# imironhead/ml_super_resolution

Hardware: AMD Instinct MI355X
Metric: VDSR-20 training patches/sec (41x41, batch 256 per GPU); fwd HR megapixels/sec alongside (higher is better)
Workload: dtype f32; 1 GPU; BASELINE configs[2]: VDSR 20-layer 3x3x64 residual, RGB, batch 256x41x41 per GPU, fwd+bwd+TF-Adam, random-init weights; global_batch=256, patch=41, parallelism=dp1

## Files before the change

### include/srx.h

```cpp
#ifndef SRX_H_
#define SRX_H_

#include <stddef.h>
#include <stdint.h>

#ifdef __cplusplus
extern "C" {
#endif

typedef void* srx_stream_t;

typedef enum {
    SRX_OK = 0,
    SRX_ERR_BAD_ARG = -1,
    SRX_ERR_UNSUPPORTED = -2,
    SRX_ERR_WORKSPACE = -3,
    SRX_ERR_LAUNCH = -4,
    SRX_ERR_ALIGN = -5
} srx_status;

typedef enum { SRX_PAD_SAME = 0, SRX_PAD_VALID = 1 } srx_pad_mode;

typedef enum {
    SRX_ACT_NONE = 0,
// ... 17 lines not shown
    int32_t subpixel_r;
} srx_conv_desc;

const char* srx_version(void);
const char* srx_last_error(void);

int srx_set_conv_path(int pipelined);

int srx_set_wgrad_path(int path);

int srx_conv_chain(const srx_conv_desc* d, int op, int in_act, int layers, const float* const* x, const float* const* w,
                   const float* const* bias, const float* const* aux, float* const* y, srx_stream_t stream);

int srx_conv_chain_supported(const srx_conv_desc* d, int op, int in_act);

int srx_set_chain(int on);

int srx_conv2d_precision_supported(const srx_conv_desc* d, int op);

size_t srx_conv2d_workspace_bytes(const srx_conv_desc* d, int op);

int srx_conv2d_fwd(const srx_conv_desc* d, const float* x, const float* w, const float* bias,
                   const float* skip, float* y, void* ws, size_t ws_bytes, srx_stream_t stream);

int srx_conv2d_bwd_data(const srx_conv_desc* d, const float* dpre, const float* w,
                        const float* x_in, int in_act, float* dx_out, void* ws, size_t ws_bytes,
                        srx_stream_t stream);

int srx_conv2d_bwd_data_acc(const srx_conv_desc* d, const float* dpre, const float* w, const float* dx_acc,
                            float* dx_out, void* ws, size_t ws_bytes, srx_stream_t stream);

// ... 163 lines not shown
```

### ml_super_resolution_amd/_lib.py

```python
import ctypes
import os

_HERE = os.path.dirname(os.path.abspath(__file__))
LIB_PATH = os.path.join(_HERE, 'libsrx.so')

SRX_OK = 0
PAD_SAME, PAD_VALID = 0, 1
ACT_NONE, ACT_RELU, ACT_TANH, ACT_LRELU, ACT_SIGMOID = 0, 1, 2, 3, 4
OP_FWD, OP_BWD_DATA, OP_BWD_FILTER = 0, 1, 2
PRECISION_FP32, PRECISION_BF16X3 = 0, 1
PRECISION_BY_NAME = {'highest': PRECISION_FP32, 'high': PRECISION_BF16X3}

ACT_BY_NAME = {None: ACT_NONE, 'none': ACT_NONE, 'relu': ACT_RELU, 'tanh': ACT_TANH,
               'lrelu': ACT_LRELU, 'leaky_relu': ACT_LRELU, 'sigmoid': ACT_SIGMOID}
PAD_BY_NAME = {'same': PAD_SAME, 'valid': PAD_VALID}

EXPORTS = [
    'srx_version', 'srx_last_error', 'srx_set_conv_path', 'srx_set_wgrad_path', 'srx_set_chain', 'srx_conv_chain', 'srx_conv_chain_supported', 'srx_conv2d_precision_supported', 'srx_conv2d_workspace_bytes', 'srx_conv2d_fwd',
    'srx_conv2d_bwd_data', 'srx_conv2d_bwd_filter', 'srx_conv2d_bwd_filter_partials', 'srx_conv2d_bwd_filter_reduce', 'srx_act_bwd', 'srx_depth_to_space',
    'srx_space_to_depth', 'srx_stream_copy', 'srx_mse_fwd_bwd', 'srx_l2_loss', 'srx_reduce_scratch_bytes',
    'srx_adam_tf_step', 'srx_adam_tf_step_dev', 'srx_momentum_clip_step', 'srx_rownorm_loss_fwd_bwd', 'srx_psnr', 'srx_ssim', 'srx_ssim_scratch_bytes', 'srx_saturate_u8', 'srx_affine', 'srx_u8_to_unit_float', 'srx_gaussian_blur', 'srx_resize_bilinear',
    'srx_upsample_nearest', 'srx_upsample_nearest_bwd', 'srx_add_relu_grad',
    'srx_conv2d_bwd_data_acc', 'srx_conv3x3_blocked', 'srx_conv3x3_blocked_bwd_filter_workspace_bytes', 'srx_conv3x3_blocked_bwd_filter',
    'srx_conv3x3_blocked_ex', 'srx_conv3x3_blocked_bwd_filter_ex_workspace_bytes', 'srx_conv3x3_blocked_bwd_filter_ex',
    'srx_espcn_forward', 'srx_espcn_forward_keep', 'srx_debug_poison_lds', 'srx_srcnn_forward', 'srx_maxpool2x2', 'srx_maxpool2x2_bwd', 'srx_maxpool2x2_bwd_masked', 'srx_subsample2', 'srx_subsample2_bwd',
    'srx_channel_blocks_to_nhwc', 'srx_nhwc_to_channel_blocks', 'srx_channel_normalize', 'srx_channel_normalize_bwd',
    'srx_extract_patches16', 'srx_texture_gram', 'srx_texture_gram_bwd', 'srx_pil_resample_ksize', 'srx_pil_resample_coeffs', 'srx_resample_u8', 'srx_u8_to_pm1', 'srx_log_loss', 'srx_vgg_preprocess', 'srx_add_scaled', 'srx_resize_bicubic_tf', 'srx_column_sums', 'srx_gemm_workspace_bytes', 'srx_gemm',
]


class SrxError(RuntimeError):
    pass

# ... 22 lines not shown
    if not os.path.exists(LIB_PATH):
        raise SrxError('libsrx.so not found at %s -- build it with `make -C %s` (or '
                       '__graft_entry__.build()); there is no CPU fallback' %
                       (LIB_PATH, os.path.join(_HERE, 'csrc')))
    import torch
    L = ctypes.CDLL(LIB_PATH)
    vp, sz, i, f = ctypes.c_void_p, ctypes.c_size_t, ctypes.c_int, ctypes.c_float
    dp = ctypes.POINTER(ConvDesc)
    L.srx_version.restype = ctypes.c_char_p
    L.srx_last_error.restype = ctypes.c_char_p
    L.srx_set_conv_path.argtypes = [i]
    L.srx_set_wgrad_path.argtypes = [i]
    L.srx_set_chain.argtypes = [i]
    L.srx_conv_chain_supported.argtypes = [dp, i, i]
    L.srx_conv_chain.argtypes = [dp, i, i, i, vp, vp, vp, vp, vp, vp]
    L.srx_conv2d_precision_supported.argtypes = [dp, i]
    L.srx_conv2d_workspace_bytes.argtypes = [dp, i]
    L.srx_conv2d_workspace_bytes.restype = sz
    L.srx_reduce_scratch_bytes.restype = sz
    L.srx_conv2d_fwd.argtypes = [dp, vp, vp, vp, vp, vp, vp, sz, vp]
    L.srx_conv2d_bwd_data.argtypes = [dp, vp, vp, vp, i, vp, vp, sz, vp]
    L.srx_conv2d_bwd_filter.argtypes = [dp, vp, vp, vp, vp, vp, f, vp, sz, vp]
    L.srx_conv2d_bwd_filter_partials.argtypes = [dp, vp, vp, vp, sz, ctypes.POINTER(ctypes.c_int), vp]
    L.srx_conv2d_bwd_filter_reduce.argtypes = [dp, vp, i, vp, vp, vp, f, vp]
    L.srx_act_bwd.argtypes = [vp, vp, vp, sz, i, vp]
    L.srx_depth_to_space.argtypes = [vp, vp, i, i, i, i, i, vp]
    L.srx_space_to_depth.argtypes = [vp, vp, i, i, i, i, i, vp]
    L.srx_stream_copy.argtypes = [vp, vp, sz, vp]
    L.srx_mse_fwd_bwd.argtypes = [vp, vp, sz, f, vp, i, vp, vp, vp]
    L.srx_l2_loss.argtypes = [vp, vp, sz, f, vp, i, vp, vp]
# ... 63 lines not shown
```

### ml_super_resolution_amd/csrc/conv_chain.hip

```cpp
#include "launchers.h"
namespace srx {

template <bool WT, int AUX>
__global__ __launch_bounds__(256, 1) void conv_chain_kernel(const ConvArgs a, const ChainPtrs c) {
    for (int l = 0; l < c.L; ++l) {
        ConvArgs al = a;
        al.x = c.x[l]; al.w = c.w[l]; al.bias = c.bias[l]; al.y = c.y[l];
        if (WT) al.mask = c.aux[l];
        else al.skip = c.aux[l];
        asm volatile("" : "+s"(al.N), "+s"(al.H), "+s"(al.W), "+s"(al.OH), "+s"(al.OW), "+s"(al.Cin), "+s"(al.Cout));
        asm volatile("" : "+s"(al.pad_t), "+s"(al.pad_l), "+s"(al.TH), "+s"(al.TW), "+s"(al.NTX), "+s"(al.RS));
        asm volatile("" : "+s"(al.units_total), "+s"(al.act), "+s"(al.post_relu), "+s"(al.mask_act), "+s"(al.buf_floats));
        conv_pipe_body<3, 3, 64, 4, WT, AUX, false>(al, l == 0);
        asm volatile("s_waitcnt vmcnt(0)" ::: "memory");
        __builtin_amdgcn_fence(__ATOMIC_RELEASE, "workgroup");
        __builtin_amdgcn_s_barrier();
        __builtin_amdgcn_fence(__ATOMIC_ACQUIRE, "workgroup");
    }
}

hipError_t launch_conv_chain(bool wt, bool aux, const ConvArgs& a, const ChainPtrs& c, int grid, size_t lds, hipStream_t s) {
    if (!wt) return aux ? hipErrorInvalidValue : launch_chain_with_lds(conv_chain_kernel<false, 0>, a, c, grid, lds, s);
    return aux ? launch_chain_with_lds(conv_chain_kernel<true, 1>, a, c, grid, lds, s)
               : launch_chain_with_lds(conv_chain_kernel<true, 0>, a, c, grid, lds, s);
}
}
```

### ml_super_resolution_amd/csrc/conv_kernels.hip.h

```cpp
#pragma once
#include <hip/hip_runtime.h>
#include <stdint.h>
#include <type_traits>

namespace srx {

typedef float f32x4 __attribute__((ext_vector_type(4)));

enum { ACT_NONE = 0, ACT_RELU = 1, ACT_TANH = 2, ACT_LRELU = 3, ACT_SIGMOID = 4 };

struct ConvArgs {
    const float* x;
    const float* w;
    const float* bias;
    const float* skip;
    const float* mask;
    float* y;
    int N, H, W, OH, OW, Cin, Cout;
    int pad_t, pad_l;
    int TH, TW, NTX, RS;
    int units_total;
    int act, post_relu, mask_act;
    float inv_rs;
    int stagger;
// ... 19 lines not shown
    float inv_rs;
    int stagger;
    int zero_slot;
    int stride;
    unsigned long long* trace;
};

constexpr int kChainMax = 32;
struct ChainPtrs {
    const float* x[kChainMax];
    const float* w[kChainMax];
    const float* bias[kChainMax];
    const float* aux[kChainMax];
    float* y[kChainMax];
    int L;
};

template <int CINP>
struct Lds {
    static constexpr int PS = (CINP == 4) ? 4 : CINP + 4;
};

__device__ __forceinline__ float srx_tanhf(float x) {
    const float ax = fabsf(x);
    const float x2 = ax * ax;
    float p = fmaf(x2, -0.006274174898862839f, 0.021071631461381912f);
    p = fmaf(x2, p, -0.053852297365665436f);
    p = fmaf(x2, p, 0.13332585990428925f);
    p = fmaf(x2, p, -0.33333316445350647f);
    const float small = fmaf(x2 * ax, p, ax);
// ... 2415 lines not shown
        }
    }
    bsum += __shfl_xor(bsum, 16);
    bsum += __shfl_xor(bsum, 32);
    if (qpart == 0 && kq == 0 && co_ok) pw[(size_t)TAPS * a.Cin * a.Cout + co] = bsum;
}

template <int IMM>
__device__ __forceinline__ float dpre_fire_imm(__amdgpu_buffer_rsrc_t rsrc, int voff, int soff) {
    float b;
    asm volatile("buffer_load_dword %0, %1, %2, %3 offen offset:%4" : "=&a"(b) : "v"(voff), "s"(rsrc), "s"(soff), "n"(IMM) : "memory");
    return b;
}

template <int KH, int KW, int CINP, int NCH, int OWC>
__global__ __launch_bounds__(256, 1) void wgrad_rows_full_kernel(const WgradArgs a) {
    extern __shared__ __attribute__((aligned(16))) float lds[];
    constexpr int PS = Lds<CINP>::PS;
    constexpr int TAPS = KH * KW;
    constexpr int ROWS = TAPS * CINP;
    constexpr int Q = (ROWS + 63) / 64;
    constexpr int NQP = 4 / NCH;
    constexpr int QW = (Q + NQP - 1) / NQP;
    constexpr int TPP = CINP / 4, PPP = 256 / TPP;
    constexpr int SPR = OWC / 4;
    constexpr int THC = 3;
    constexpr int RSZ = OWC + 1;
    constexpr int COUTC = 64;
    constexpr int U = THC * SPR + 1;
    constexpr int JP = (RSZ + PPP - 1) / PPP;
    constexpr int NPASSES = (THC + KH - 1) * JP;
// ... 229 lines not shown
#pragma unroll
        for (int g = 0; g < 4; ++g) {
#pragma unroll
            for (int r = 0; r < 4; ++r) {
                const int R = 64 * q + 4 * (4 * kq + r) + g;
                const int tap = R / CINP, ci = R % CINP;
                if (R < ROWS && ci < a.Cin && co_ok) pw[((size_t)tap * a.Cin + ci) * a.Cout + co] = acc[k][g][r];
            }
        }
    }
    bsum += __shfl_xor(bsum, 16);
    bsum += __shfl_xor(bsum, 32);
    if (qpart == 0 && kq == 0 && co_ok) pw[(size_t)TAPS * a.Cin * a.Cout + co] = bsum;
}

}
```

### ml_super_resolution_amd/csrc/launchers.h

```cpp
#pragma once
#include "conv_kernels.hip.h"

namespace srx {

struct ConvKey {
    int kh, kw, cinp, nch;
    bool wt;
};

bool launch_conv_k3c64(const ConvKey& k, const ConvArgs& a, int grid, size_t lds, hipStream_t s, hipError_t* err);
bool launch_conv_k3c32(const ConvKey& k, const ConvArgs& a, int grid, size_t lds, hipStream_t s, hipError_t* err);
bool launch_conv_c4(const ConvKey& k, const ConvArgs& a, int grid, size_t lds, hipStream_t s, hipError_t* err);
bool launch_conv_misc(const ConvKey& k, const ConvArgs& a, int grid, size_t lds, hipStream_t s, hipError_t* err);
bool launch_pipe_k3c64(const ConvKey& k, const ConvArgs& a, int grid, size_t lds, hipStream_t s, hipError_t* err);
bool launch_pipe_other(const ConvKey& k, const ConvArgs& a, int grid, size_t lds, hipStream_t s, hipError_t* err);
bool launch_wgrad_narrow(const ConvKey& k, const WgradArgs& a, int grid, hipStream_t s, hipError_t* err);
bool launch_conv_narrow(const ConvKey& k, const ConvArgs& a, hipStream_t s, hipError_t* err);
bool launch_conv_1x1(const ConvKey& k, const ConvArgs& a, long min_pixels, hipStream_t s, hipError_t* err);
bool launch_conv_rows3x3(const ConvKey& k, const ConvArgs& a, long min_pixels, hipStream_t s, hipError_t* err);
bool launch_conv_pack3(const ConvKey& k, const ConvArgs& a, long min_pixels, hipStream_t s, hipError_t* err);
bool launch_conv_kwrows(const ConvKey& k, const ConvArgs& a, long min_pixels, hipStream_t s, hipError_t* err);
bool launch_pipe_strip(const ConvKey& k, const ConvArgs& a, int grid, size_t lds, hipStream_t s, hipError_t* err);
bool launch_conv_generic(const ConvKey& k, const ConvArgs& a, int grid, size_t lds, hipStream_t s, hipError_t* err);
bool launch_wgrad(const ConvKey& k, const WgradArgs& a, int grid, size_t lds, hipStream_t s, hipError_t* err);
bool launch_wgrad_generic(const ConvKey& k, const WgradArgs& a, int grid, size_t lds, hipStream_t s, hipError_t* err);
bool launch_wgrad_lin(const ConvKey& k, const WgradArgs& a, int grid, size_t lds, hipStream_t s, hipError_t* err);
bool launch_wgrad_lin_pack3(const ConvKey& k, const WgradArgs& a, int grid, size_t lds, hipStream_t s, hipError_t* err);
bool launch_wgrad_lin_strip(const ConvKey& k, const WgradArgs& a, int grid, size_t lds, hipStream_t s, hipError_t* err);
bool launch_wgrad_pipe(const ConvKey& k, const WgradArgs& a, int grid, size_t lds, hipStream_t s, hipError_t* err);
bool launch_wgrad_kwcols(const ConvKey& k, const WgradArgs& a, int max_partials, long min_pixels, int* n_partials, hipStream_t s, hipError_t* err);
bool launch_wgrad_1x1(const ConvKey& k, const WgradArgs& a, int max_partials, int* n_partials, hipStream_t s, hipError_t* err);
bool launch_wgrad_rows_full(const ConvKey& k, const WgradArgs& a, int grid, size_t lds, hipStream_t s, hipError_t* err);
bool launch_wgrad_rows_strip(const ConvKey& k, const WgradArgs& a, int grid, size_t lds, bool nt, hipStream_t s, hipError_t* err);
bool launch_wgrad_lin_pairs(const ConvKey& k, const WgradPairs& q, int grid, int pairs, bool strips, size_t lds, hipStream_t s, hipError_t* err);

__attribute__((weak)) hipError_t launch_conv_chain(bool wt, bool aux, const ConvArgs& a, const ChainPtrs& c, int grid, size_t lds, hipStream_t s);

hipError_t launch_reduce_partials(const float* part, int G, int stride, int wn, int cout, float* dw, float* dbias,
                                  const float* w, float wd, hipStream_t s);
hipError_t launch_reduce_partials_pairs(const float* part, int G, int stride, int wn, int cout, float* dw, float* dbias,
                                        int pairs, int cob, hipStream_t s);

template <typename K, typename A>
inline hipError_t launch_with_lds(K kernel, const A& a, int grid, size_t lds, hipStream_t s, int grid_y = 1) {
    static thread_local const void* configured[64];
    static thread_local int n_configured = 0;
    const void* fn = reinterpret_cast<const void*>(kernel);
    bool known = false;
    for (int i = 0; i < n_configured; ++i) known |= (configured[i] == fn);
    if (!known) {
        hipError_t e = hipFuncSetAttribute(fn, hipFuncAttributeMaxDynamicSharedMemorySize, 160 * 1024);
// ... 98 lines not shown
```

### ml_super_resolution_amd/csrc/srx_api.hip

```cpp
#include <math.h>
#include <stdarg.h>
#include <atomic>
#include <stdio.h>
#include <stdlib.h>
#include <string.h>

#include "../../include/srx.h"
#include "elementwise.h"
#include "launchers.h"
#include "bf16x3.h"

using namespace srx;

namespace {

thread_local char g_err[512] = "";

struct Knobs {
    int pipe_default, min_full_th, small_rule, th, grid, narrow, dyn, stagger, wgrad_lin, wgrad_pipe, wgrad_pipe_strip, wgrad_rows_full, wgrad_1x1, wgrad_pack3, wgrad_nt, kwrows_min_pixels, big_route_min_pixels, strip_d2s, conv_1x1_min_pixels, pack3_dgrad;
    int subpixel_chunk_kb, subpixel_db, subpixel_grid, subpixel_depth, subpixel_throttle, subpixel_even;
    int chain;
    unsigned long long* trace;
    int dbg;
};
int env_int(const char* name, int dflt) { const char* e = getenv(name); return e ? atoi(e) : dflt; }
Knobs read_knobs() {
    Knobs k;
    k.pipe_default = env_int("SRX_PIPE", 1);
    k.min_full_th = env_int("SRX_MIN_FULL_TH", 3);
    k.small_rule = env_int("SRX_SMALL_RULE", 1);
    k.th = env_int("SRX_TH", -1);
    k.grid = env_int("SRX_GRID", -1);
    k.narrow = env_int("SRX_NARROW", 1);
    k.dyn = env_int("SRX_DYN", 0);
    k.stagger = env_int("SRX_STAGGER", -1);
    k.wgrad_lin = env_int("SRX_WGRAD_LIN", 1);
// ... 3 lines not shown
    k.big_route_min_pixels = env_int("SRX_BIG_ROUTE_MIN_PIXELS", 60000);
    k.conv_1x1_min_pixels = env_int("SRX_CONV_1X1_MIN_PIXELS", 100000);
    k.pack3_dgrad = env_int("SRX_PACK3_DGRAD", 1);
    k.strip_d2s = env_int("SRX_STRIP_D2S", 1);
    k.wgrad_rows_full = env_int("SRX_WGRAD_ROWS_FULL", 1);
    k.wgrad_1x1 = env_int("SRX_WGRAD_1X1", 1);
    k.wgrad_pack3 = env_int("SRX_WGRAD_PACK3", 1);
    k.wgrad_nt = env_int("SRX_WGRAD_NT", 1);
    k.subpixel_chunk_kb = env_int("SRX_SUBPIXEL_CHUNK_KB", 24);
    k.subpixel_db = env_int("SRX_SUBPIXEL_DB", 1);
    k.subpixel_grid = env_int("SRX_SUBPIXEL_GRID", 0);
    k.subpixel_depth = env_int("SRX_SUBPIXEL_DEPTH", 0);
    k.subpixel_throttle = env_int("SRX_SUBPIXEL_THROTTLE", -1);
    k.subpixel_even = env_int("SRX_SUBPIXEL_EVEN", 1);
    k.chain = env_int("SRX_CHAIN", 1);
    k.trace = nullptr;
    k.dbg = 0;
#ifdef SRX_TRACE
    { const char* tp = getenv("SRX_TRACE_PTR"); k.trace = tp ? (unsigned long long*)strtoull(tp, nullptr, 0) : nullptr; }
    k.dbg = env_int("SRX_DBG", 0);
#endif
    return k;
}
const Knobs& knobs() { static const Knobs k = read_knobs(); return k; }

std::atomic<int> g_use_pipe{-1};
std::atomic<int> g_chain{-1};
int use_chain() { const int v = g_chain.load(std::memory_order_relaxed); return v < 0 ? (knobs().chain ? 1 : 0) : v; }
int use_pipe() { const int v = g_use_pipe.load(std::memory_order_relaxed); return v < 0 ? knobs().pipe_default : v; }
std::atomic<int> g_wgrad_path{-1};
int wgrad_path_default() { return !knobs().wgrad_lin ? 0 : ((knobs().wgrad_pipe || knobs().wgrad_pipe_strip) ? 2 : 1); }
int wgrad_path() { const int v = g_wgrad_path.load(std::memory_order_relaxed); return v < 0 ? wgrad_path_default() : v; }

int cu_count() {
    static std::atomic<int> cached[64];
    int dev = 0;
    if (hipGetDevice(&dev) != hipSuccess || dev < 0 || dev >= 64) { (void)hipGetLastError(); return 256; }
    int n = cached[dev].load(std::memory_order_relaxed);
    if (n > 0) return n;
    if (hipDeviceGetAttribute(&n, hipDeviceAttributeMultiprocessorCount, dev) != hipSuccess || n <= 0) {
        (void)hipGetLastError();
        n = 256;
    }
// ... 535 lines not shown
        return SRX_OK;
    }
    int pt, pl, OH, OW;
    geometry(d, &pt, &pl, &OH, &OW);
    Plan p;
    rc = make_plan(d->N, OH, OW, d->H, d->W, d->Cout, d->Cin, d->KH, d->KW, d->KH - 1 - pt, d->KW - 1 - pl, &p);
    if (rc) return rc;
    ConvArgs a;
    memset(&a, 0, sizeof(a));
    a.x = dpre; a.w = w; a.bias = nullptr; a.skip = dx_acc; a.mask = x_in; a.y = dx_out;
    fill_conv_args(&a, p, d->N, OH, OW, d->Cout, d->Cin);
    a.act = SRX_ACT_NONE; a.post_relu = 0; a.mask_act = in_act;
    return dispatch_conv(p, true, a, (hipStream_t)stream, ws, ws_bytes);
}

static void wgrad_tile_for_linear_walk(const srx_conv_desc* d, Plan* p) {
    if (p->NTX != 1 || wgrad_path() < 1) return;
    const size_t slot_bytes = (size_t)((p->cinp == 4) ? 4 : p->cinp + 4) * 4;
    while (p->TH > 1 && p->lds_bytes + 4 * slot_bytes > 80 * 1024) {
        p->TH -= 1;
        p->lds_bytes = ((size_t)(p->TH + d->KH - 1) * p->RS + (d->KW - 1)) * slot_bytes;
    }
}

int srx_conv2d_bwd_filter_partials(const srx_conv_desc* d, const float* x, const float* dpre, void* ws, size_t ws_bytes,
                                   int* n_partials, srx_stream_t stream) {
    int rc = check_desc(d);
    if (rc) return rc;
    if (!x || !dpre || !n_partials) return fail(SRX_ERR_BAD_ARG, "null tensor pointer");
    if (!aligned16(x) || !aligned16(dpre)) return fail(SRX_ERR_ALIGN, "tensor base pointers must be 16-byte aligned");
    if (d->precision == SRX_PRECISION_BF16X3) {
        if ((rc = bf16x3_supported(d, SRX_OP_BWD_FILTER)) != SRX_OK) return rc;
        Bf3Plan bp;
        bf16x3_plan(d->N, d->H, d->W, max_grid(), true, &bp);
        const size_t need = (size_t)bp.grid * part_stride(d) * sizeof(float);
        if (!ws || ws_bytes < need) return fail(SRX_ERR_WORKSPACE, "bwd_filter needs %zu workspace bytes, got %zu", need, ws_bytes);
        if (!aligned16(ws)) return fail(SRX_ERR_ALIGN, "workspace must be 16-byte aligned");
        const hipError_t err = launch_wgrad3x3c64_bf16x3(x, dpre, (float*)ws, (int)part_stride(d), d->N, d->H, d->W, bp, (hipStream_t)stream);
// ... 2 lines not shown
        return SRX_OK;
    }
    int pt, pl, OH, OW;
    geometry(d, &pt, &pl, &OH, &OW);
    Plan p;
    const bool s2 = d->stride == 2;
    rc = s2 ? make_plan_s2(d->N, d->H, d->W, OH, OW, d->Cin, d->Cout, d->KH, d->KW, pt, pl, &p)
            : make_plan(d->N, d->H, d->W, OH, OW, d->Cin, d->Cout, d->KH, d->KW, pt, pl, &p);
    if (rc) return rc;
    if (!s2) wgrad_tile_for_linear_walk(d, &p);
    const size_t need = (size_t)p.grid * part_stride(d) * sizeof(float);
    if (!ws || ws_bytes < need)
        return fail(SRX_ERR_WORKSPACE, "bwd_filter needs %zu workspace bytes, got %zu", need, ws_bytes);
    if (!aligned16(ws)) return fail(SRX_ERR_ALIGN, "workspace must be 16-byte aligned");
    WgradArgs a;
    memset(&a, 0, sizeof(a));
    a.x = x; a.dpre = dpre;
    a.part = (float*)ws;
    a.part_stride = (int)part_stride(d);
    a.N = d->N; a.H = d->H; a.W = d->W; a.OH = OH; a.OW = OW; a.Cin = d->Cin; a.Cout = d->Cout;
    a.pad_t = pt; a.pad_l = pl; a.TH = p.TH; a.TW = p.TW; a.NTX = p.NTX; a.RS = p.RS;
    a.units_total = p.units_total; a.inv_rs = 1.0f / (float)p.RS;
    a.stagger = stagger_sleeps(p);
    a.stride = d->stride;
    a.zero_slot = ((p.TH - 1) * d->stride + d->KH) * p.RS + (d->KW - 1);
    a.trace = knobs().trace;
    const size_t wg_lds = p.lds_bytes + (size_t)((p.cinp == 4) ? 4 : p.cinp + 4) * 4;
    ConvKey k{d->KH, d->KW, p.cinp, p.nch, false};
    hipError_t err = hipSuccess;
    hipStream_t s = (hipStream_t)stream;
    const int wpath = wgrad_path();
    const int use_lin = wpath >= 1 && !s2;
    const int kPipeGrid = pipe_grid();
    const bool lin_ok = use_lin && p.NTX == 1 && OW >= 4 && p.RS >= 8 && p.RS == d->W + pl && (long)p.TH * OW * d->Cout * 4 < (1L << 30) &&
                        (long)d->H * d->W * d->Cin * 4 < (1L << 31) - 4096;
    const size_t lin_lds = p.lds_bytes + 4 * (size_t)((p.cinp == 4) ? 4 : p.cinp + 4) * 4;
    const int use_wpipe = wpath >= 2 && knobs().wgrad_pipe;
    const int wppp = (p.cinp >= 16) ? 256 / (p.cinp / 4) : 256;
    int wgrid = p.grid;
    bool wdone = false;
    if (knobs().wgrad_1x1 && wpath >= 1 && !s2) {
        int n1 = 0;
        if (launch_wgrad_1x1(k, a, p.grid, &n1, s, &err)) { wdone = true; wgrid = n1; }
    }
    if (!wdone && knobs().big_route_min_pixels >= 0 && wpath >= 1 && !s2) {
        int n1 = 0;
        if (launch_wgrad_kwcols(k, a, p.grid, knobs().big_route_min_pixels, &n1, s, &err)) { wdone = true; wgrid = n1; }
    }
    if (!wdone && use_wpipe && knobs().wgrad_rows_full && lin_ok && d->KH == 3 && d->KW == 3 && d->Cin == 64 && d->Cout == 64 && OW == 41 && d->W == 41 &&
        pl == 1 && pt == 1 && p.RS == 42) {
        WgradArgs ap = a;
        ap.TH = 3;
        ap.zero_slot = (3 + 3) * 42 + 2;
        wgrid = p.grid < kPipeGrid ? p.grid : kPipeGrid;
        wdone = launch_wgrad_rows_full(k, ap, wgrid, 2 * (size_t)(ap.zero_slot + 4) * (64 + 4) * 4, s, &err);
        if (!wdone) wgrid = p.grid;
    }
    if (!wdone && use_wpipe && lin_ok && d->Cin == p.cinp && p.RS >= wppp && 2 * lin_lds <= 160 * 1024) {
        const int kWin = 14 * 4;
        int best_th = 0;
        double best_waste = 1e9;
        for (int th = p.TH; th >= 1; --th) {
            const long pos = (long)th * p.RS, padded = (pos + kWin - 1) / kWin * kWin;
            const double waste = (double)(padded - pos) / (double)pos;
            const bool fits = padded + 2L * p.RS + 6 <= (long)a.zero_slot + 4;
            if (fits && waste < best_waste - 1e-9) { best_waste = waste; best_th = th; }
        }
        if (best_th > 0 && best_waste <= 0.10) {
            WgradArgs ap = a;
            ap.TH = best_th;
// ... 37 lines not shown
    if (n_partials <= 0 || n_partials > kMaxGridLimit) return fail(SRX_ERR_BAD_ARG, "bad partial count %d", n_partials);
    const size_t wn = (size_t)d->KH * d->KW * d->Cin * d->Cout;
    hipError_t err = launch_reduce_partials((const float*)ws, n_partials, (int)part_stride(d), (int)wn, d->Cout, dw, dbias,
                                            w_for_decay, wd_scale, (hipStream_t)stream);
    if (err != hipSuccess) return fail(SRX_ERR_LAUNCH, "reduce launch failed: %s", hipGetErrorString(err));
    return SRX_OK;
}

int srx_conv2d_bwd_filter(const srx_conv_desc* d, const float* x, const float* dpre, float* dw, float* dbias,
                          const float* w_for_decay, float wd_scale, void* ws, size_t ws_bytes, srx_stream_t stream) {
    if (!dw) return fail(SRX_ERR_BAD_ARG, "null tensor pointer");
    int n = 0;
    const int rc = srx_conv2d_bwd_filter_partials(d, x, dpre, ws, ws_bytes, &n, stream);
    if (rc) return rc;
    return srx_conv2d_bwd_filter_reduce(d, ws, n, dw, dbias, w_for_decay, wd_scale, stream);
}

namespace {
void blocked_desc(srx_conv_desc* d, int N, int H, int W) {
    memset(d, 0, sizeof(*d));
    d->N = N; d->H = H; d->W = W; d->Cin = 64; d->Cout = 64; d->KH = 3; d->KW = 3; d->stride = 1; d->pad_mode = SRX_PAD_SAME;
}
int pairs_route(const srx_conv_desc* d, const Plan& p, int pairs, int* G, size_t* lin_lds) {
    *lin_lds = p.lds_bytes + 4 * (size_t)(p.cinp + 4) * 4;
    const bool common = wgrad_path() >= 1 && p.cinp == 64 && p.nch == 4 && d->W >= 4 && p.RS >= 8 && *lin_lds <= 80 * 1024 &&
                        (long)d->H * d->W * 64 * 4 < (1L << 31) - 4096;
    const bool lin_ok = common && p.NTX == 1 && p.RS == d->W + p.pad_l && (long)p.TH * d->W * 64 * 4 < (1L << 30);
    const int wppp = 256 / (64 / 4);
    const bool strip_ok = common && p.NTX > 1 && p.RS >= wppp && p.TW >= 4 && (d->W % p.TW == 0 || d->W % p.TW >= 4) &&
                          p.RS <= 3 * wppp && (long)d->H * d->W * 64 * 4 < (1L << 30);
// ... 318 lines not shown
```

### ml_super_resolution_amd/csrc/wgrad_inst.hip

```cpp
#include "launchers.h"
namespace srx {
__device__ __forceinline__ void reduce_partials_body(const float* __restrict__ part, int G, int stride, int wn, int n,
                                                     float* __restrict__ dw, float* __restrict__ dbias,
                                                     const float* __restrict__ w, float wd) {
    __shared__ f32x4 sh[16][17];
    const int c = threadIdx.x & 15, pg = threadIdx.x >> 4;
    const int j = blockIdx.x * 64 + 4 * c;
    f32x4 s = {0.f, 0.f, 0.f, 0.f};
    if (j < n) {
        const float* p = part + j;
        int g = pg;
        for (; g + 7 * 16 < G; g += 8 * 16) {
            f32x4 v[8];
#pragma unroll
            for (int i = 0; i < 8; ++i) v[i] = *reinterpret_cast<const f32x4*>(p + (size_t)(g + 16 * i) * stride);
#pragma unroll
            for (int i = 0; i < 8; ++i) s += v[i];
        }
        for (; g < G; g += 16) s += *reinterpret_cast<const f32x4*>(p + (size_t)g * stride);
    }
    sh[pg][c] = s;
    __syncthreads();
    if (pg == 0 && j < n) {
        f32x4 t = sh[0][c];
// ... 10 lines not shown
    }
}

__global__ __launch_bounds__(256) void reduce_partials_kernel(const float* __restrict__ part, int G, int stride,
                                                              int wn, int n, float* __restrict__ dw,
                                                              float* __restrict__ dbias, const float* __restrict__ w,
                                                              float wd) {
    reduce_partials_body(part, G, stride, wn, n, dw, dbias, w, wd);
}
__global__ __launch_bounds__(256) void reduce_partials_pairs_kernel(const float* __restrict__ part, int G, int stride,
                                                                    int wn, int n, float* __restrict__ dw,
                                                                    float* __restrict__ dbias, int cob) {
    const int pair = blockIdx.y;
    float* db = (dbias && pair < cob) ? dbias + (size_t)pair * (n - wn) : nullptr;
    reduce_partials_body(part + (size_t)pair * G * stride, G, stride, wn, n, dw + (size_t)pair * wn, db, nullptr, 0.f);
}

hipError_t launch_reduce_partials_pairs(const float* part, int G, int stride, int wn, int cout, float* dw, float* dbias,
                                        int pairs, int cob, hipStream_t s) {
    const int n = wn + cout;
    hipLaunchKernelGGL(reduce_partials_pairs_kernel, dim3((unsigned)((n + 63) / 64), (unsigned)pairs), dim3(256), 0, s, part, G,
                       stride, wn, n, dw, dbias, cob);
    return hipGetLastError();
}

hipError_t launch_reduce_partials(const float* part, int G, int stride, int wn, int cout, float* dw, float* dbias,
                                  const float* w, float wd, hipStream_t s) {
    const int n = wn + cout;
    hipLaunchKernelGGL(reduce_partials_kernel, dim3((unsigned)((n + 63) / 64)), dim3(256), 0, s, part, G, stride, wn, n,
                       dw, dbias, w, wd);
// ... 43 lines not shown
```

### ml_super_resolution_amd/engine.py

```python
import math
import os

import torch

from . import ops


class LayerSpec(object):

    def __init__(self, ksize, cin, cout, padding='same', act=None, scope=None):
        self.kh, self.kw = (ksize, ksize) if isinstance(ksize, int) else ksize
        self.cin, self.cout = cin, cout
        self.padding = padding.lower()
        self.act = act
        self.scope = scope

    @property
    def kernel_shape(self):
        return (self.kh, self.kw, self.cin, self.cout)

    def out_hw(self, h, w):
        if self.padding == 'same':
            return h, w
        return h - self.kh + 1, w - self.kw + 1
# ... 190 lines not shown
            row_len = y.shape[1] * y.shape[2]
            dy = ops.rownorm_loss_fwd_bwd(y, target, row_len, self.loss, dpred=self._buf(('dy', 0), y.shape),
                                          norms=self._buf(('rownorms',), (y.numel() // row_len,)))
        else:
            dy = self._buf(('dy', 0), y.shape)
            ops.mse_fwd_bwd(y, target, self.loss, inv_numel=inv, accumulate=False, dpred=dy)
        if self.weight_decay:
            self.add_regulariser_loss()
        if self.specs[last].act is not None:
            dpre = ops.act_bwd(dy, y, self.specs[last].act, out=self._buf(('dpre_last',), y.shape))
        else:
            dpre = dy
        prec = self.layer_precision
        need = max(ops.bwd_filter_workspace_bytes(acts[i].shape, s.kernel_shape, s.padding, precision=prec[i])
                   for i, s in enumerate(self.specs))
        if self._ws is None or self._ws.numel() * 4 < need:
            self._step_graphs.clear()
            self._ws = torch.empty((need + 3) // 4, dtype=torch.float32, device=self.device)
            self._ws2 = None
        main = torch.cuda.current_stream(self.device) if self.device.type == 'cuda' else None
        two = self.overlap_wgrad and main is not None
        if two and self._side is None:
            self._side = torch.cuda.Stream(device=self.device)
        red = self.overlap_reduce and main is not None and not two
        if red:
            if self._side is None:
                self._side = torch.cuda.Stream(device=self.device)
            if self._ws2 is None or self._ws2.numel() != self._ws.numel():
                self._ws2 = torch.empty_like(self._ws)
        ws_free = [None, None]
        read_done = {}
        chain = None if (two or red) else self._dgrad_chain(acts)
        for i in range(last, -1, -1):
            s = self.specs[i]
            if chain is not None and chain[0] <= i <= chain[1]:
                lo, hi = chain
                if i == hi:
                    outs = [self._buf(('dpre_chain', k - 1), acts[k].shape) for k in range(hi, lo - 1, -1)]
                    ops.conv2d_bwd_data_chain([dpre] + outs[:-1], [self.kernel(k) for k in range(hi, lo - 1, -1)],
                                              [acts[k] for k in range(hi, lo - 1, -1)], outs, acts[hi].shape, s.padding,
                                              in_act=self.specs[hi - 1].act)
                    dpres = {hi: dpre}
                    for k in range(hi, lo - 1, -1):
                        dpres[k - 1] = outs[hi - k]
                ops.conv2d_bwd_filter(acts[i], dpres[i], s.kernel_shape, s.padding,
                                      w_for_decay=self.kernel(i) if self.weight_decay else None,
                                      wd_scale=self.weight_decay, dw=self.kernel(i, self.grads),
                                      dbias=self.bias(i, self.grads), workspace=self._ws, precision=prec[i])
                if i == lo:
                    dpre = dpres[lo - 1]
                continue
            if red:
                k = i & 1
                ws = self._ws if k == 0 else self._ws2
                if ws_free[k] is not None:
                    main.wait_event(ws_free[k])
                n_part = ops.conv2d_bwd_filter_partials(acts[i], dpre, s.kernel_shape, s.padding, ws, precision=prec[i])
                ready = torch.cuda.Event()
                ready.record(main)
                with torch.cuda.stream(self._side):
                    self._side.wait_event(ready)
                    ops.conv2d_bwd_filter_reduce(acts[i].shape, s.kernel_shape, s.padding, ws, n_part,
                                                 self.kernel(i, self.grads), self.bias(i, self.grads),
# ... 226 lines not shown
```

### ml_super_resolution_amd/ops.py

```python
import ctypes
import os

import torch

from . import _lib
from ._lib import ACT_BY_NAME, PAD_BY_NAME, ConvDesc, check
from ._lib import lib as _load_lib

_POISON_LDS = os.environ.get('SRX_POISON_LDS', '0') == '1'


def lib():
    L = _load_lib()
    if _POISON_LDS and torch.cuda.is_available():
        L.srx_debug_poison_lds(_stream())
    return L



def _stream():
    return ctypes.c_void_p(torch.cuda.current_stream().cuda_stream)


def _ptr(t):
# ... 120 lines not shown
    for l in range(len(dpres)):
        _chk(dpres[l], 'dpre'); _chk(ws[l], 'w'); _chk(outs[l], 'out')
        if masks is not None:
            _chk(masks[l], 'x_in')
        if tuple(outs[l].shape) != tuple(x_shape) or tuple(ws[l].shape) != tuple(ws[0].shape) or tuple(dpres[l].shape) != tuple(dpres[0].shape):
            raise ValueError('conv2d_bwd_data_chain: layer %d does not have the shape of layer 0' % l)
    d = conv_desc(x_shape, ws[0].shape, padding)
    check(lib().srx_conv_chain(ctypes.byref(d), _lib.OP_BWD_DATA, ACT_BY_NAME[in_act] if masks is not None else _lib.ACT_NONE, len(dpres),
                               _ptr_array(dpres), _ptr_array(ws), None, None if masks is None else _ptr_array(masks),
                               _ptr_array(outs), _stream()), 'srx_conv_chain')
    return outs[-1]


def set_chain(on):
    return lib().srx_set_chain(int(on))


def bwd_filter_workspace_bytes(x_shape, w_shape, padding='same', stride=1, precision='highest'):
    d = conv_desc(x_shape, w_shape, padding, stride=stride, precision=precision)
    return lib().srx_conv2d_workspace_bytes(ctypes.byref(d), _lib.OP_BWD_FILTER)


def conv2d_bwd_filter(x, dpre, w_shape, padding='same', w_for_decay=None, wd_scale=0.0, dw=None, dbias=None,
                      want_dbias=True, workspace=None, stride=1, precision='highest'):
    for t, n in ((x, 'x'), (dpre, 'dpre'), (w_for_decay, 'w_for_decay')):
        _chk(t, n)
    d = conv_desc(x.shape, w_shape, padding, stride=stride, precision=precision)
    if tuple(dpre.shape) != tuple(out_shape(d)):
        raise ValueError('dpre has shape %s, the layer output is %s' % (tuple(dpre.shape), tuple(out_shape(d))))
    if dw is None:
# ... 553 lines not shown
```

Baseline: 18870 patches/s.

## Chain per-layer filter-gradient kernels into one persistent launch plus batched reduce

Adds a chained weight-gradient path for the run of identical 3x3 64->64 layers. One persistent kernel loops over all layers with the full-row wgrad body, and a single reduce kernel uses one grid row per layer. This replaces per-layer partial and reduce launches, cutting launch and tail overhead, at the cost of a workspace that grows with the layer count. It applies only when the wgrad/reduce overlap is off, so it may drop any side-stream overlap of the reduce.

```diff
diff --git a/include/srx.h b/include/srx.h
--- a/include/srx.h
+++ b/include/srx.h
@@ -55,7 +55,17 @@
 
 int srx_conv_chain_supported(const srx_conv_desc* d, int op, int in_act);
 
+int srx_conv_chain_bwd_filter(const srx_conv_desc* d, int layers, const float* const* x, const float* const* dpre, void* ws,
+                              size_t ws_bytes, float* const* dw, float* const* dbias, const float* const* w_for_decay,
+                              float wd_scale, srx_stream_t stream);
+
+int srx_conv_chain_bwd_filter_supported(const srx_conv_desc* d);
+
+size_t srx_conv_chain_bwd_filter_workspace_bytes(const srx_conv_desc* d, int layers);
+
 int srx_set_chain(int on);
+
+int srx_set_wgrad_chain(int on);
 
 int srx_conv2d_precision_supported(const srx_conv_desc* d, int op);
 
diff --git a/ml_super_resolution_amd/_lib.py b/ml_super_resolution_amd/_lib.py
--- a/ml_super_resolution_amd/_lib.py
+++ b/ml_super_resolution_amd/_lib.py
@@ -16,7 +16,7 @@
 PAD_BY_NAME = {'same': PAD_SAME, 'valid': PAD_VALID}
 
 EXPORTS = [
-    'srx_version', 'srx_last_error', 'srx_set_conv_path', 'srx_set_wgrad_path', 'srx_set_chain', 'srx_conv_chain', 'srx_conv_chain_supported', 'srx_conv2d_precision_supported', 'srx_conv2d_workspace_bytes', 'srx_conv2d_fwd',
+    'srx_version', 'srx_last_error', 'srx_set_conv_path', 'srx_set_wgrad_path', 'srx_set_chain', 'srx_conv_chain', 'srx_conv_chain_supported', 'srx_conv_chain_bwd_filter', 'srx_conv_chain_bwd_filter_supported', 'srx_conv_chain_bwd_filter_workspace_bytes', 'srx_set_wgrad_chain', 'srx_conv2d_precision_supported', 'srx_conv2d_workspace_bytes', 'srx_conv2d_fwd',
     'srx_conv2d_bwd_data', 'srx_conv2d_bwd_filter', 'srx_conv2d_bwd_filter_partials', 'srx_conv2d_bwd_filter_reduce', 'srx_act_bwd', 'srx_depth_to_space',
     'srx_space_to_depth', 'srx_stream_copy', 'srx_mse_fwd_bwd', 'srx_l2_loss', 'srx_reduce_scratch_bytes',
     'srx_adam_tf_step', 'srx_adam_tf_step_dev', 'srx_momentum_clip_step', 'srx_rownorm_loss_fwd_bwd', 'srx_psnr', 'srx_ssim', 'srx_ssim_scratch_bytes', 'srx_saturate_u8', 'srx_affine', 'srx_u8_to_unit_float', 'srx_gaussian_blur', 'srx_resize_bilinear',
@@ -69,6 +69,11 @@
     L.srx_set_chain.argtypes = [i]
     L.srx_conv_chain_supported.argtypes = [dp, i, i]
     L.srx_conv_chain.argtypes = [dp, i, i, i, vp, vp, vp, vp, vp, vp]
+    L.srx_conv_chain_bwd_filter.argtypes = [dp, i, vp, vp, vp, sz, vp, vp, vp, f, vp]
+    L.srx_conv_chain_bwd_filter_supported.argtypes = [dp]
+    L.srx_conv_chain_bwd_filter_workspace_bytes.argtypes = [dp, i]
+    L.srx_conv_chain_bwd_filter_workspace_bytes.restype = sz
+    L.srx_set_wgrad_chain.argtypes = [i]
     L.srx_conv2d_precision_supported.argtypes = [dp, i]
     L.srx_conv2d_workspace_bytes.argtypes = [dp, i]
     L.srx_conv2d_workspace_bytes.restype = sz
diff --git a/ml_super_resolution_amd/csrc/conv_chain.hip b/ml_super_resolution_amd/csrc/conv_chain.hip
--- a/ml_super_resolution_amd/csrc/conv_chain.hip
+++ b/ml_super_resolution_amd/csrc/conv_chain.hip
@@ -19,6 +19,29 @@
     }
 }
 
+__global__ __launch_bounds__(256, 1) void wgrad_chain_kernel(const WgradArgs a, const WgradChainPtrs c) {
+    for (int l = 0; l < c.L; ++l) {
+        WgradArgs al = a;
+        al.x = c.x[l]; al.dpre = c.dpre[l]; al.part = c.part[l];
+        asm volatile("" : "+s"(al.N), "+s"(al.H), "+s"(al.W), "+s"(al.OH), "+s"(al.OW), "+s"(al.Cin), "+s"(al.Cout));
+        asm volatile("" : "+s"(al.pad_t), "+s"(al.pad_l), "+s"(al.TH), "+s"(al.TW), "+s"(al.NTX), "+s"(al.RS));
+        asm volatile("" : "+s"(al.units_total), "+s"(al.part_stride), "+s"(al.zero_slot), "+s"(al.stagger), "+s"(al.stride));
+        wgrad_rows_full_body<3, 3, 64, 4, 41>(al);
+    }
+}
+
+hipError_t launch_wgrad_chain(const WgradArgs& a, const WgradChainPtrs& c, int grid, size_t lds, hipStream_t s) {
+    static thread_local bool configured = false;
+    if (!configured) {
+        const hipError_t e = hipFuncSetAttribute(reinterpret_cast<const void*>(wgrad_chain_kernel),
+                                                 hipFuncAttributeMaxDynamicSharedMemorySize, 160 * 1024);
+        if (e != hipSuccess) return e;
+        configured = true;
+    }
+    hipLaunchKernelGGL(wgrad_chain_kernel, dim3(grid), dim3(256), lds, s, a, c);
+    return hipGetLastError();
+}
+
 hipError_t launch_conv_chain(bool wt, bool aux, const ConvArgs& a, const ChainPtrs& c, int grid, size_t lds, hipStream_t s) {
     if (!wt) return aux ? hipErrorInvalidValue : launch_chain_with_lds(conv_chain_kernel<false, 0>, a, c, grid, lds, s);
     return aux ? launch_chain_with_lds(conv_chain_kernel<true, 1>, a, c, grid, lds, s)
diff --git a/ml_super_resolution_amd/csrc/conv_kernels.hip.h b/ml_super_resolution_amd/csrc/conv_kernels.hip.h
--- a/ml_super_resolution_amd/csrc/conv_kernels.hip.h
+++ b/ml_super_resolution_amd/csrc/conv_kernels.hip.h
@@ -57,6 +57,17 @@
     const float* aux[kChainMax];
     float* y[kChainMax];
     int L;
+};
+struct WgradChainPtrs {
+    const float* x[kChainMax];
+    const float* dpre[kChainMax];
+    float* part[kChainMax];
+    int L;
+};
+struct ReduceChainPtrs {
+    float* dw[kChainMax];
+    float* dbias[kChainMax];
+    const float* w[kChainMax];
 };
 
 template <int CINP>
@@ -2502,7 +2513,7 @@
 }
 
 template <int KH, int KW, int CINP, int NCH, int OWC>
-__global__ __launch_bounds__(256, 1) void wgrad_rows_full_kernel(const WgradArgs a) {
+__device__ __forceinline__ void wgrad_rows_full_body(const WgradArgs a) {
     extern __shared__ __attribute__((aligned(16))) float lds[];
     constexpr int PS = Lds<CINP>::PS;
     constexpr int TAPS = KH * KW;
@@ -2762,4 +2773,9 @@
     if (qpart == 0 && kq == 0 && co_ok) pw[(size_t)TAPS * a.Cin * a.Cout + co] = bsum;
 }
 
-}
+template <int KH, int KW, int CINP, int NCH, int OWC>
+__global__ __launch_bounds__(256, 1) void wgrad_rows_full_kernel(const WgradArgs a) {
+    wgrad_rows_full_body<KH, KW, CINP, NCH, OWC>(a);
+}
+
+}
diff --git a/ml_super_resolution_amd/csrc/launchers.h b/ml_super_resolution_amd/csrc/launchers.h
--- a/ml_super_resolution_amd/csrc/launchers.h
+++ b/ml_super_resolution_amd/csrc/launchers.h
@@ -35,6 +35,10 @@
 bool launch_wgrad_lin_pairs(const ConvKey& k, const WgradPairs& q, int grid, int pairs, bool strips, size_t lds, hipStream_t s, hipError_t* err);
 
 __attribute__((weak)) hipError_t launch_conv_chain(bool wt, bool aux, const ConvArgs& a, const ChainPtrs& c, int grid, size_t lds, hipStream_t s);
+
+__attribute__((weak)) hipError_t launch_wgrad_chain(const WgradArgs& a, const WgradChainPtrs& c, int grid, size_t lds, hipStream_t s);
+__attribute__((weak)) hipError_t launch_reduce_partials_chain(const float* part, size_t layer_floats, int layers, int G, int stride, int wn, int cout,
+                                        const ReduceChainPtrs& r, float wd, hipStream_t s);
 
 hipError_t launch_reduce_partials(const float* part, int G, int stride, int wn, int cout, float* dw, float* dbias,
                                   const float* w, float wd, hipStream_t s);
diff --git a/ml_super_resolution_amd/csrc/srx_api.hip b/ml_super_resolution_amd/csrc/srx_api.hip
--- a/ml_super_resolution_amd/csrc/srx_api.hip
+++ b/ml_super_resolution_amd/csrc/srx_api.hip
@@ -19,7 +19,7 @@
 struct Knobs {
     int pipe_default, min_full_th, small_rule, th, grid, narrow, dyn, stagger, wgrad_lin, wgrad_pipe, wgrad_pipe_strip, wgrad_rows_full, wgrad_1x1, wgrad_pack3, wgrad_nt, kwrows_min_pixels, big_route_min_pixels, strip_d2s, conv_1x1_min_pixels, pack3_dgrad;
     int subpixel_chunk_kb, subpixel_db, subpixel_grid, subpixel_depth, subpixel_throttle, subpixel_even;
-    int chain;
+    int chain, wgrad_chain, wgrad_chain_reduce;
     unsigned long long* trace;
     int dbg;
 };
@@ -53,6 +53,8 @@
     k.subpixel_throttle = env_int("SRX_SUBPIXEL_THROTTLE", -1);
     k.subpixel_even = env_int("SRX_SUBPIXEL_EVEN", 1);
     k.chain = env_int("SRX_CHAIN", 1);
+    k.wgrad_chain = env_int("SRX_WGRAD_CHAIN", 1);
+    k.wgrad_chain_reduce = env_int("SRX_WGRAD_CHAIN_REDUCE", 1);
     k.trace = nullptr;
     k.dbg = 0;
 #ifdef SRX_TRACE
@@ -66,6 +68,8 @@
 std::atomic<int> g_use_pipe{-1};
 std::atomic<int> g_chain{-1};
 int use_chain() { const int v = g_chain.load(std::memory_order_relaxed); return v < 0 ? (knobs().chain ? 1 : 0) : v; }
+std::atomic<int> g_wgrad_chain{-1};
+int use_wgrad_chain() { const int v = g_wgrad_chain.load(std::memory_order_relaxed); return v < 0 ? (knobs().wgrad_chain ? 1 : 0) : v; }
 int use_pipe() { const int v = g_use_pipe.load(std::memory_order_relaxed); return v < 0 ? knobs().pipe_default : v; }
 std::atomic<int> g_wgrad_path{-1};
 int wgrad_path_default() { return !knobs().wgrad_lin ? 0 : ((knobs().wgrad_pipe || knobs().wgrad_pipe_strip) ? 2 : 1); }
@@ -631,6 +635,18 @@
     return dispatch_conv(p, true, a, (hipStream_t)stream, ws, ws_bytes);
 }
 
+static void fill_wgrad_args(WgradArgs* a, const srx_conv_desc* d, const Plan& p, int pt, int pl, int OH, int OW) {
+    memset(a, 0, sizeof(*a));
+    a->part_stride = (int)part_stride(d);
+    a->N = d->N; a->H = d->H; a->W = d->W; a->OH = OH; a->OW = OW; a->Cin = d->Cin; a->Cout = d->Cout;
+    a->pad_t = pt; a->pad_l = pl; a->TH = p.TH; a->TW = p.TW; a->NTX = p.NTX; a->RS = p.RS;
+    a->units_total = p.units_total; a->inv_rs = 1.0f / (float)p.RS;
+    a->stagger = stagger_sleeps(p);
+    a->stride = d->stride;
+    a->zero_slot = ((p.TH - 1) * d->stride + d->KH) * p.RS + (d->KW - 1);
+    a->trace = knobs().trace;
+}
+
 static void wgrad_tile_for_linear_walk(const srx_conv_desc* d, Plan* p) {
     if (p->NTX != 1 || wgrad_path() < 1) return;
     const size_t slot_bytes = (size_t)((p->cinp == 4) ? 4 : p->cinp + 4) * 4;
@@ -639,6 +655,15 @@
         p->lds_bytes = ((size_t)(p->TH + d->KH - 1) * p->RS + (d->KW - 1)) * slot_bytes;
     }
 }
+
+static bool rows_full_shape(const srx_conv_desc* d, const Plan& p, int pt, int pl, int OW) {
+    return d->KH == 3 && d->KW == 3 && d->Cin == 64 && d->Cout == 64 && OW == 41 && d->W == 41 && pl == 1 && pt == 1 && p.RS == 42;
+}
+static void rows_full_args(WgradArgs* a) {
+    a->TH = 3;
+    a->zero_slot = (3 + 3) * 42 + 2;
+}
+static size_t rows_full_lds(const WgradArgs& a) { return 2 * (size_t)(a.zero_slot + 4) * (64 + 4) * 4; }
 
 int srx_conv2d_bwd_filter_partials(const srx_conv_desc* d, const float* x, const float* dpre, void* ws, size_t ws_bytes,
                                    int* n_partials, srx_stream_t stream) {
@@ -671,17 +696,9 @@
         return fail(SRX_ERR_WORKSPACE, "bwd_filter needs %zu workspace bytes, got %zu", need, ws_bytes);
     if (!aligned16(ws)) return fail(SRX_ERR_ALIGN, "workspace must be 16-byte aligned");
     WgradArgs a;
-    memset(&a, 0, sizeof(a));
+    fill_wgrad_args(&a, d, p, pt, pl, OH, OW);
     a.x = x; a.dpre = dpre;
     a.part = (float*)ws;
-    a.part_stride = (int)part_stride(d);
-    a.N = d->N; a.H = d->H; a.W = d->W; a.OH = OH; a.OW = OW; a.Cin = d->Cin; a.Cout = d->Cout;
-    a.pad_t = pt; a.pad_l = pl; a.TH = p.TH; a.TW = p.TW; a.NTX = p.NTX; a.RS = p.RS;
-    a.units_total = p.units_total; a.inv_rs = 1.0f / (float)p.RS;
-    a.stagger = stagger_sleeps(p);
-    a.stride = d->stride;
-    a.zero_slot = ((p.TH - 1) * d->stride + d->KH) * p.RS + (d->KW - 1);
-    a.trace = knobs().trace;
     const size_t wg_lds = p.lds_bytes + (size_t)((p.cinp == 4) ? 4 : p.cinp + 4) * 4;
     ConvKey k{d->KH, d->KW, p.cinp, p.nch, false};
     hipError_t err = hipSuccess;
@@ -704,13 +721,11 @@
         int n1 = 0;
         if (launch_wgrad_kwcols(k, a, p.grid, knobs().big_route_min_pixels, &n1, s, &err)) { wdone = true; wgrid = n1; }
     }
-    if (!wdone && use_wpipe && knobs().wgrad_rows_full && lin_ok && d->KH == 3 && d->KW == 3 && d->Cin == 64 && d->Cout == 64 && OW == 41 && d->W == 41 &&
-        pl == 1 && pt == 1 && p.RS == 42) {
+    if (!wdone && use_wpipe && knobs().wgrad_rows_full && lin_ok && rows_full_shape(d, p, pt, pl, OW)) {
         WgradArgs ap = a;
-        ap.TH = 3;
-        ap.zero_slot = (3 + 3) * 42 + 2;
+        rows_full_args(&ap);
         wgrid = p.grid < kPipeGrid ? p.grid : kPipeGrid;
-        wdone = launch_wgrad_rows_full(k, ap, wgrid, 2 * (size_t)(ap.zero_slot + 4) * (64 + 4) * 4, s, &err);
+        wdone = launch_wgrad_rows_full(k, ap, wgrid, rows_full_lds(ap), s, &err);
         if (!wdone) wgrid = p.grid;
     }
     if (!wdone && use_wpipe && lin_ok && d->Cin == p.cinp && p.RS >= wppp && 2 * lin_lds <= 160 * 1024) {
@@ -778,6 +793,101 @@
     const int rc = srx_conv2d_bwd_filter_partials(d, x, dpre, ws, ws_bytes, &n, stream);
     if (rc) return rc;
     return srx_conv2d_bwd_filter_reduce(d, ws, n, dw, dbias, w_for_decay, wd_scale, stream);
+}
+
+}
+namespace {
+int wgrad_chain_plan(const srx_conv_desc* d, WgradArgs* a, int* grid, size_t* lds) {
+    int rc = check_desc(d);
+    if (rc) return rc;
+    if (!use_chain()) return fail(SRX_ERR_UNSUPPORTED, "wgrad chain: switched off (srx_set_chain / SRX_CHAIN)");
+    if (!use_wgrad_chain()) return fail(SRX_ERR_UNSUPPORTED, "wgrad chain: switched off (srx_set_wgrad_chain / SRX_WGRAD_CHAIN)");
+    if (!launch_wgrad_chain || !launch_reduce_partials_chain) return fail(SRX_ERR_UNSUPPORTED, "wgrad chain: this build has no chain kernels");
+    if (d->precision != SRX_PRECISION_FP32) return fail(SRX_ERR_UNSUPPORTED, "wgrad chain: precision %d (exact fp32 only)", d->precision);
+    if (d->KH != 3 || d->KW != 3 || d->Cin != 64 || d->Cout != 64 || d->stride != 1 || d->pad_mode != SRX_PAD_SAME)
+        return fail(SRX_ERR_UNSUPPORTED, "wgrad chain: only 3x3 64->64 stride-1 SAME layers");
+    if (d->W != 41) return fail(SRX_ERR_UNSUPPORTED, "wgrad chain: W %d (41-pixel rows only)", d->W);
+    if (wgrad_path() < 2 || !knobs().wgrad_pipe || !knobs().wgrad_rows_full)
+        return fail(SRX_ERR_UNSUPPORTED, "wgrad chain: filter-gradient path %d does not take wgrad_rows_full_kernel", wgrad_path());
+    int pt, pl, OH, OW;
+    geometry(d, &pt, &pl, &OH, &OW);
+    Plan p;
+    rc = make_plan(d->N, d->H, d->W, OH, OW, d->Cin, d->Cout, d->KH, d->KW, pt, pl, &p);
+    if (rc) return rc;
+    wgrad_tile_for_linear_walk(d, &p);
+    const bool lin_ok = p.NTX == 1 && OW >= 4 && p.RS >= 8 && p.RS == d->W + pl && (long)p.TH * OW * d->Cout * 4 < (1L << 30) &&
+                        (long)d->H * d->W * d->Cin * 4 < (1L << 31) - 4096;
+    if (!lin_ok || !rows_full_shape(d, p, pt, pl, OW))
+        return fail(SRX_ERR_UNSUPPORTED, "wgrad chain: the shape is not on the full-width 41-pixel-row route");
+    *grid = p.grid < pipe_grid() ? p.grid : pipe_grid();
+    if (d->N % *grid) return fail(SRX_ERR_UNSUPPORTED, "wgrad chain: N %d is not a multiple of the grid %d", d->N, *grid);
+    fill_wgrad_args(a, d, p, pt, pl, OH, OW);
+    rows_full_args(a);
+    a->trace = nullptr;
+    *lds = rows_full_lds(*a);
+    return SRX_OK;
+}
+}
+extern "C" {
+
+int srx_set_wgrad_chain(int on) {
+    const int old = g_wgrad_chain.exchange(on < 0 ? -1 : (on ? 1 : 0), std::memory_order_relaxed);
+    return old < 0 ? (knobs().wgrad_chain ? 1 : 0) : old;
+}
+
+int srx_conv_chain_bwd_filter_supported(const srx_conv_desc* d) {
+    WgradArgs a;
+    int grid;
+    size_t lds;
+    return wgrad_chain_plan(d, &a, &grid, &lds) == SRX_OK ? 1 : 0;
+}
+
+size_t srx_conv_chain_bwd_filter_workspace_bytes(const srx_conv_desc* d, int layers) {
+    if (layers < 1 || layers > kChainMax) return 0;
+    WgradArgs a;
+    int grid;
+    size_t lds;
+    if (wgrad_chain_plan(d, &a, &grid, &lds) != SRX_OK) return 0;
+    return (size_t)layers * grid * a.part_stride * sizeof(float);
+}
+
+int srx_conv_chain_bwd_filter(const srx_conv_desc* d, int layers, const float* const* x, const float* const* dpre, void* ws,
+                              size_t ws_bytes, float* const* dw, float* const* dbias, const float* const* w_for_decay,
+                              float wd_scale, srx_stream_t stream) {
+    if (layers < 1 || layers > kChainMax) return fail(SRX_ERR_BAD_ARG, "wgrad chain: %d layers (1..%d)", layers, kChainMax);
+    if (!x || !dpre || !dw) return fail(SRX_ERR_BAD_ARG, "null pointer array");
+    WgradArgs a;
+    int grid;
+    size_t lds;
+    const int rc = wgrad_chain_plan(d, &a, &grid, &lds);
+    if (rc) return rc;
+    const size_t layer_floats = (size_t)grid * a.part_stride;
+    const size_t need = (size_t)layers * layer_floats * sizeof(float);
+    if (!ws || ws_bytes < need) return fail(SRX_ERR_WORKSPACE, "wgrad chain needs %zu workspace bytes, got %zu", need, ws_bytes);
+    if (!aligned16(ws)) return fail(SRX_ERR_ALIGN, "workspace must be 16-byte aligned");
+    WgradChainPtrs c;
+    ReduceChainPtrs r;
+    memset(&c, 0, sizeof(c));
+    memset(&r, 0, sizeof(r));
+    c.L = layers;
+    for (int l = 0; l < layers; ++l) {
+        if (!x[l] || !dpre[l] || !dw[l]) return fail(SRX_ERR_BAD_ARG, "wgrad chain: null tensor pointer in layer %d", l);
+        if (!aligned16(x[l]) || !aligned16(dpre[l])) return fail(SRX_ERR_ALIGN, "tensor base pointers must be 16-byte aligned");
+        c.x[l] = x[l]; c.dpre[l] = dpre[l]; c.part[l] = (float*)ws + l * layer_floats;
+        r.dw[l] = dw[l]; r.dbias[l] = dbias ? dbias[l] : nullptr; r.w[l] = w_for_decay ? w_for_decay[l] : nullptr;
+    }
+    hipStream_t s = (hipStream_t)stream;
+    hipError_t err = launch_wgrad_chain(a, c, grid, lds, s);
+    if (err != hipSuccess) return fail(SRX_ERR_LAUNCH, "wgrad chain launch failed: %s", hipGetErrorString(err));
+    const int wn = 3 * 3 * 64 * 64;
+    if (knobs().wgrad_chain_reduce) {
+        err = launch_reduce_partials_chain((const float*)ws, layer_floats, layers, grid, a.part_stride, wn, 64, r, wd_scale, s);
+    } else {
+        for (int l = 0; l < layers && err == hipSuccess; ++l)
+            err = launch_reduce_partials(c.part[l], grid, a.part_stride, wn, 64, r.dw[l], r.dbias[l], r.w[l], wd_scale, s);
+    }
+    if (err != hipSuccess) return fail(SRX_ERR_LAUNCH, "reduce launch failed: %s", hipGetErrorString(err));
+    return SRX_OK;
 }
 
 namespace {
diff --git a/ml_super_resolution_amd/csrc/wgrad_inst.hip b/ml_super_resolution_amd/csrc/wgrad_inst.hip
--- a/ml_super_resolution_amd/csrc/wgrad_inst.hip
+++ b/ml_super_resolution_amd/csrc/wgrad_inst.hip
@@ -48,6 +48,20 @@
     const int pair = blockIdx.y;
     float* db = (dbias && pair < cob) ? dbias + (size_t)pair * (n - wn) : nullptr;
     reduce_partials_body(part + (size_t)pair * G * stride, G, stride, wn, n, dw + (size_t)pair * wn, db, nullptr, 0.f);
+}
+
+__global__ __launch_bounds__(256) void reduce_partials_chain_kernel(const float* __restrict__ part, size_t layer_floats, int G,
+                                                                    int stride, int wn, int n, const ReduceChainPtrs r, float wd) {
+    const int l = blockIdx.y;
+    reduce_partials_body(part + (size_t)l * layer_floats, G, stride, wn, n, r.dw[l], r.dbias[l], r.w[l], wd);
+}
+
+hipError_t launch_reduce_partials_chain(const float* part, size_t layer_floats, int layers, int G, int stride, int wn, int cout,
+                                        const ReduceChainPtrs& r, float wd, hipStream_t s) {
+    const int n = wn + cout;
+    hipLaunchKernelGGL(reduce_partials_chain_kernel, dim3((unsigned)((n + 63) / 64), (unsigned)layers), dim3(256), 0, s, part,
+                       layer_floats, G, stride, wn, n, r, wd);
+    return hipGetLastError();
 }
 
 hipError_t launch_reduce_partials_pairs(const float* part, int G, int stride, int wn, int cout, float* dw, float* dbias,
diff --git a/ml_super_resolution_amd/engine.py b/ml_super_resolution_amd/engine.py
--- a/ml_super_resolution_amd/engine.py
+++ b/ml_super_resolution_amd/engine.py
@@ -228,6 +228,15 @@
         prec = self.layer_precision
         need = max(ops.bwd_filter_workspace_bytes(acts[i].shape, s.kernel_shape, s.padding, precision=prec[i])
                    for i, s in enumerate(self.specs))
+        chain = None if ((self.overlap_wgrad or self.overlap_reduce) and self.device.type == 'cuda') else self._dgrad_chain(acts)
+        wchain = False
+        if chain is not None:
+            lo, hi = chain
+            s = self.specs[hi]
+            wneed = ops.bwd_filter_chain_workspace_bytes(acts[hi].shape, s.kernel_shape, hi - lo + 1, s.padding)
+            if wneed > 0:
+                wchain = True
+                need = max(need, wneed)
         if self._ws is None or self._ws.numel() * 4 < need:
             self._step_graphs.clear()
             self._ws = torch.empty((need + 3) // 4, dtype=torch.float32, device=self.device)
@@ -244,7 +253,6 @@
                 self._ws2 = torch.empty_like(self._ws)
         ws_free = [None, None]
         read_done = {}
-        chain = None if (two or red) else self._dgrad_chain(acts)
         for i in range(last, -1, -1):
             s = self.specs[i]
             if chain is not None and chain[0] <= i <= chain[1]:
@@ -257,10 +265,18 @@
                     dpres = {hi: dpre}
                     for k in range(hi, lo - 1, -1):
                         dpres[k - 1] = outs[hi - k]
-                ops.conv2d_bwd_filter(acts[i], dpres[i], s.kernel_shape, s.padding,
-                                      w_for_decay=self.kernel(i) if self.weight_decay else None,
-                                      wd_scale=self.weight_decay, dw=self.kernel(i, self.grads),
-                                      dbias=self.bias(i, self.grads), workspace=self._ws, precision=prec[i])
+                    if wchain:
+                        ks = range(hi, lo - 1, -1)
+                        ops.conv2d_bwd_filter_chain([acts[k] for k in ks], [dpres[k] for k in ks],
+                                                    [self.kernel(k, self.grads) for k in ks], [self.bias(k, self.grads) for k in ks],
+                                                    self._ws, s.padding,
+                                                    ws_for_decay=[self.kernel(k) for k in ks] if self.weight_decay else None,
+                                                    wd_scale=self.weight_decay)
+                if not wchain:
+                    ops.conv2d_bwd_filter(acts[i], dpres[i], s.kernel_shape, s.padding,
+                                          w_for_decay=self.kernel(i) if self.weight_decay else None,
+                                          wd_scale=self.weight_decay, dw=self.kernel(i, self.grads),
+                                          dbias=self.bias(i, self.grads), workspace=self._ws, precision=prec[i])
                 if i == lo:
                     dpre = dpres[lo - 1]
                 continue
diff --git a/ml_super_resolution_amd/ops.py b/ml_super_resolution_amd/ops.py
--- a/ml_super_resolution_amd/ops.py
+++ b/ml_super_resolution_amd/ops.py
@@ -158,6 +158,41 @@
 
 def set_chain(on):
     return lib().srx_set_chain(int(on))
+
+
+def set_wgrad_chain(on):
+    return lib().srx_set_wgrad_chain(int(on))
+
+
+def bwd_filter_chain_supported(x_shape, w_shape, padding='same', precision='highest'):
+    d = conv_desc(x_shape, w_shape, padding, precision=precision)
+    return lib().srx_conv_chain_bwd_filter_supported(ctypes.byref(d)) == 1
+
+
+def bwd_filter_chain_workspace_bytes(x_shape, w_shape, layers, padding='same'):
+    d = conv_desc(x_shape, w_shape, padding)
+    return int(lib().srx_conv_chain_bwd_filter_workspace_bytes(ctypes.byref(d), int(layers)))
+
+
+def conv2d_bwd_filter_chain(xs, dpres, dws, dbiases, workspace, padding='same', ws_for_decay=None, wd_scale=0.0):
+    n = len(xs)
+    if len(dpres) != n or len(dws) != n or (dbiases is not None and len(dbiases) != n) or (ws_for_decay is not None and len(ws_for_decay) != n):
+        raise ValueError('conv2d_bwd_filter_chain: per-layer lists of different lengths')
+    for l in range(n):
+        _chk(xs[l], 'x'); _chk(dpres[l], 'dpre'); _chk(dws[l], 'dw')
+        if dbiases is not None:
+            _chk(dbiases[l], 'dbias')
+        if ws_for_decay is not None:
+            _chk(ws_for_decay[l], 'w_for_decay')
+        if tuple(xs[l].shape) != tuple(xs[0].shape) or tuple(dpres[l].shape) != tuple(dpres[0].shape) or tuple(dws[l].shape) != tuple(dws[0].shape):
+            raise ValueError('conv2d_bwd_filter_chain: layer %d does not have the shape of layer 0' % l)
+    _chk(workspace, 'workspace')
+    d = conv_desc(xs[0].shape, dws[0].shape, padding)
+    check(lib().srx_conv_chain_bwd_filter(ctypes.byref(d), n, _ptr_array(xs), _ptr_array(dpres), _ptr(workspace),
+                                          workspace.numel() * workspace.element_size(), _ptr_array(dws),
+                                          None if dbiases is None else _ptr_array(dbiases),
+                                          None if ws_for_decay is None else _ptr_array(ws_for_decay),
+                                          float(wd_scale), _stream()), 'srx_conv_chain_bwd_filter')
 
 
 def bwd_filter_workspace_bytes(x_shape, w_shape, padding='same', stride=1, precision='highest'):
```

New measurement: 19060 patches/s, median of 6. 1.01x the previous value.
